# Rinoahu/SwiftOrtho

Hardware: AMD Instinct MI355X
Metric: M query-aa/s scanned all-vs-all (higher is better)
Workload: dtype u8/int16/int32 (5-bit packed residues, packed 16-bit score-only DP, int32 traced DP); 1 GPU; BASELINE config 3: 100000 synthetic proteins x 300 aa self-search, seed 11111011111, aa9, -M 120000000, -c 50000 (2 chunks), -e 1e-5, -v 500; query_aa=30007201, rows=1618760

## Files before the change

### swiftortho_amd/csrc/k_ungapq.hip

```cpp
#include "ungap1.h"

#define UQ_WAVES 16
#define UQ_RING 128
#define UQ_TBITS 12
#define UQ_QCAP 512
#define UQ_QSLOT (UQ_QCAP + 2 * U1_QPAD)
#define UQ_TILE 256
#define UQ_WAVE_BYTES (UQ_QSLOT + (1 << UQ_TBITS) / 4 + UQ_RING * 4 + UQ_RING * 4 + UQ_RING * 2 + UQ_TILE * 8)

__device__ __forceinline__ u32 bk_scan_max16(u32 x) {
    x = max(x, (u32)__builtin_amdgcn_update_dpp(0, (int)x, 0x111, 0xf, 0xf, true));
    x = max(x, (u32)__builtin_amdgcn_update_dpp(0, (int)x, 0x112, 0xf, 0xf, true));
    x = max(x, (u32)__builtin_amdgcn_update_dpp(0, (int)x, 0x114, 0xf, 0xf, true));
    x = max(x, (u32)__builtin_amdgcn_update_dpp(0, (int)x, 0x118, 0xf, 0xf, true));
    x = max(x, (u32)__builtin_amdgcn_update_dpp(0, (int)x, 0x142, 0xa, 0xf, false));
    x = max(x, (u32)__builtin_amdgcn_update_dpp(0, (int)x, 0x143, 0xc, 0xf, false));
    return x;
}

__device__ __forceinline__ u32 uq_slot(u32 g) { return (g * 2654435761u) >> (32 - UQ_TBITS); }

__global__ __launch_bounds__(256) void k_uq_first(const u32* __restrict__ qseg, u32 nqp, const u32* __restrict__ cs_hoff, u32 K, u32* __restrict__ qk) {
    const u32 q = blockIdx.x * 256u + threadIdx.x;
    if (q > nqp) return;
    const u32 x = qseg[q];
    u32 lo = 0, hi = K;
    while (lo < hi) {
        const u32 m = (lo + hi) >> 1;
        if (cs_hoff[m] < x) lo = m + 1;
        else hi = m;
    }
    qk[q] = lo;
}

template <bool BANDS, bool COUNT>
__global__ __launch_bounds__(64 * UQ_WAVES, 1) __attribute__((amdgpu_num_sgpr(96))) void k_ungapq(
    const u32* __restrict__ qseg , u32 nqp, u32 qa, const u32* __restrict__ qk, const u32* __restrict__ cs_hoff,
    const u32* __restrict__ cs_base, const u64* __restrict__ cs_kbase, const u32* __restrict__ dk32, int bp, int bd, int sh_q, int sh_qpos, int sh_diag, int diag_off, int rbs,
    int rsh_subj, int rsh_diag, int rdoff, const uint2* __restrict__ btab, u32 wait_n, const u8* __restrict__ q_scls, const u32* __restrict__ qoff,
    const u8* __restrict__ r_ug, const u32* __restrict__ roff, const signed char* __restrict__ b62g, u32* __restrict__ work_ctr, u32* __restrict__ shard_cnt,
    u64* __restrict__ p_qs, u64* __restrict__ p_sd, u64* __restrict__ p_ft, unsigned long long* __restrict__ group_count, u64* __restrict__ keys,
    u64* __restrict__ keys_sorted, u32* __restrict__ seg_end, unsigned long long* __restrict__ stat ) {
    constexpr int TSH = 3;
    constexpr u32 TBYTES = (u32)U1_ROWS << (8 + TSH);
    __shared__ __align__(16) unsigned char uq_smem[TBYTES + UQ_WAVES * UQ_WAVE_BYTES];
    const int lane = threadIdx.x & 63, w = threadIdx.x >> 6;
    for (u32 i = threadIdx.x; i < U1_ROWS * 32u * 32u; i += 64 * UQ_WAVES) {
        const u32 q = i >> 10, s = (i >> 5) & 31u, l = i & 31u;
        const int v = (q < SCLS_N && s < SCLS_N) ? (int)b62g[q * SCLS_N + s] : -100;
        *reinterpret_cast<short*>(uq_smem + ((q << 11) | (s << 6) | (l << 1))) = (short)v;
    }
    __syncthreads();
    unsigned char* wbase = uq_smem + TBYTES + (u32)w * UQ_WAVE_BYTES;
    u8* qslot = wbase;
    u32* tab = reinterpret_cast<u32*>(wbase + UQ_QSLOT);
    u32* ring_s = tab + (1 << UQ_TBITS) / 16;
    u32* ring_g = ring_s + UQ_RING;
    u16* ring_q = reinterpret_cast<u16*>(ring_g + UQ_RING);
    u32* mbase = reinterpret_cast<u32*>(ring_q + UQ_RING);
    u16* marks = reinterpret_cast<u16*>(mbase + UQ_TILE);
    u16* mqpos = marks + UQ_TILE;
    static_assert(UQ_TILE == 256, "tile_marks clears the marks with two words per lane");
    static_assert(U1_PCAP * 8 <= 7 * 64 && UQ_WAVES <= U1_ROWS, "pass buffer in a table row's tail");
    u64* s_pass = reinterpret_cast<u64*>(uq_smem + ((u32)w << 11) + 25 * 64);
    u16* s_passq = reinterpret_cast<u16*>(uq_smem + ((u32)w << 11) + 25 * 64 + U1_PCAP * 8);
    static_assert(U1_PCAP * 8 + U1_PCAP * 2 <= 7 * 64, "row tail");
    const unsigned long long lt = (1ull << lane) - 1ull;
    const u32 lanebase = (u32)(size_t)(__attribute__((address_space(3))) unsigned char*)uq_smem + ((u32)(lane & 31) << 1);
    const u32 pmask = (1u << bp) - 1u;
    const u32 dmask = (1u << bd) - 1u;
    u32 npb = 0, ngroups = 0;
    u32 ch_pos = 0, ch_end = 0;
    U1Track tr_unused;
    U1Count ct;
    ct.n = 0;
    ct.start();

    for (;;) {
        u32 qrel = 0;
        if (lane == 0) qrel = atomicAdd(work_ctr, 1u);
        qrel = (u32)__builtin_amdgcn_readfirstlane((int)qrel);
        if (qrel >= nqp) break;
        const u32 h0 = (u32)__builtin_amdgcn_readfirstlane((int)qseg[qrel]), h1 = (u32)__builtin_amdgcn_readfirstlane((int)qseg[qrel + 1]);
        if (h0 == h1) {
            if (lane == 0) seg_end[qrel] = h0;
            continue;
        }
        const u32 k0 = (u32)__builtin_amdgcn_readfirstlane((int)qk[qrel]), k1 = (u32)__builtin_amdgcn_readfirstlane((int)qk[qrel + 1]);
        const u32 gq = qa + qrel;
        const u32 qb0 = (u32)__builtin_amdgcn_readfirstlane((int)qoff[gq]);
        const int ql = (int)((u32)__builtin_amdgcn_readfirstlane((int)qoff[gq + 1]) - qb0);
        for (int i = lane * 16; i < UQ_QSLOT; i += 64 * 16) {
            const int p0 = i - U1_QPAD;
            uint4 v = make_uint4(0x18181818u, 0x18181818u, 0x18181818u, 0x18181818u);
            if (p0 >= 0 && p0 < ql) {
                v = u1_load16(q_scls + qb0 + (u32)p0);
                u32* d = reinterpret_cast<u32*>(&v);
#pragma unroll
                for (int k = 0; k < 4; ++k) {
                    const int nv = min(max(ql - p0 - 4 * k, 0), 4);
                    const u32 m = nv >= 4 ? 0xFFFFFFFFu : ((1u << (8 * nv)) - 1u);
                    d[k] = (d[k] & m) | (0x18181818u & ~m);
                }
                if (p0 == 0) d[0] = (d[0] & 0xFFFFFF00u) | 0x18u;
            }
            *reinterpret_cast<uint4*>(qslot + i) = v;
        }
        reinterpret_cast<uint4*>(tab)[lane] = make_uint4(0, 0, 0, 0);
        u1_wave_sync();
        const int qr_max = U1_QPAD + ql;
        const u64 kq = (u64)gq << sh_q;

        const u32 n = h1 - h0;
        u32 t_next = k0;
        u32 c_base = 0, c_qpos = 0;
        auto tile_marks = [&](u32 tb) {
            reinterpret_cast<u32*>(marks)[lane] = 0, reinterpret_cast<u32*>(marks)[64 + lane] = 0;
            u1_wave_sync();
            for (;;) {
                const u32 k = t_next + (u32)lane;
                u32 o = 0xFFFFFFFFu;
                if (k < k1) o = cs_hoff[k] - h0 - tb;
                const bool in = o < (u32)UQ_TILE;
                if (in) {
                    marks[o] = (u16)(o + 1u);
                    mbase[o] = cs_base[k] + h0;
                    mqpos[o] = (u16)((u32)(cs_kbase[k] >> sh_qpos) & pmask);
                }
                const u32 cnt = (u32)__popcll(__ballot(in));
                t_next += cnt;
                if (cnt < 64u) break;
            }
            u1_wave_sync();
        };
        auto gen_step = [&](u32 tb, u32 st, u32& c, u32& qpos, u32& o) -> bool {
            o = tb + 64u * st + (u32)lane;
            const u32 p1 = bk_scan_max16((u32)marks[64u * st + (u32)lane]);
            u32 base = c_base;
            qpos = c_qpos;
            if (p1) base = mbase[p1 - 1u], qpos = (u32)mqpos[p1 - 1u];
            c_base = (u32)__builtin_amdgcn_readlane((int)base, 63), c_qpos = (u32)__builtin_amdgcn_readlane((int)qpos, 63);
            c = 0xFFFFFFFFu;
            if (o >= n) return false;
            c = dk32[base + o];
            return (int)c >= 0;
        };
        for (u32 tb = 0; tb < n; tb += UQ_TILE) {
            tile_marks(tb);
            const u32 nst = (min(n - tb, (u32)UQ_TILE) + 63u) / 64u;
            for (u32 st = 0; st < nst; ++st) {
                u32 c, qpos, o;
                if (gen_step(tb, st, c, qpos, o)) {
                    const u32 t = uq_slot(c + qpos), sh = (t & 15u) * 2u;
                    const u32 old = atomicOr(&tab[t >> 4], 1u << sh);
                    if ((old >> sh) & 1u) atomicOr(&tab[t >> 4], 2u << sh);
                }
            }
        }
        u1_wave_sync();

        auto flush = [&]() {
            const u32 at = u1_reserve(npb, lane, ch_pos, ch_end, &shard_cnt[0], U1_CHUNK);
            if ((u32)lane < npb) {
                const u64 e = s_pass[lane];
                const u32 G = (u32)e, qp = (u32)s_passq[lane];
                u32 gsubj;
                int dlt;
                if (BANDS) {
                    const uint2 be = btab[G >> bd];
                    gsubj = be.x;
                    dlt = (int)(be.y - G);
                } else {
                    gsubj = G >> bd;
                    dlt = diag_off - (int)(G & dmask);
                }
                p_qs[at] = ((u64)gq << rbs) | gsubj;
                p_sd[at] = (e & 0xFFFFFFFF00000000ull) | (u64)(u32)dlt;
                p_ft[at] = ((u64)gsubj << rsh_subj) | ((u64)(u32)(rdoff - dlt) << rsh_diag) | ((u64)qp << sh_qpos);
            }
            npb = 0;
        };
        t_next = k0, c_base = 0, c_qpos = 0;
        u32 g_tb = 0, g_st = 0, g_nst = (min(n, (u32)UQ_TILE) + 63u) / 64u;
        tile_marks(0);
        bool more = true;
        u32 ns = 0;
        u32 rfront = 0, rback = 0;
        bool working = false;
        int qR = 0, qL = 0;
        i64 sR = 0, sL = 0;
        u32 hG = 0, hq = 0;
        pk16 S = {0, 0}, M = {0, 0};
        for (;;) {
            const unsigned long long idleb = __ballot(!working);
            if (idleb && ((u32)__popcll(idleb) >= wait_n || idleb == ~0ull)) {
                while (rback - rfront <= UQ_RING - 64u && more) {
                    u32 c, qpos, o;
                    const bool valid = gen_step(g_tb, g_st, c, qpos, o);
                    bool sing = false;
                    u32 G = 0;
                    if (valid) {
                        G = c + qpos;
                        const u32 t = uq_slot(G);
                        sing = ((tab[t >> 4] >> ((t & 15u) * 2u)) & 3u) == 1u;
                    }
                    const unsigned long long sb_ = __ballot(sing), kb_ = __ballot(valid && !sing);
                    if (valid && !sing) keys[h0 + ns + (u32)__popcll(kb_ & lt)] = kq + ((u64)qpos << sh_diag) + ((u64)qpos << sh_qpos) + ((u64)c << sh_diag);
                    ns += (u32)__popcll(kb_);
                    if (sing) {
                        u32 gsubj;
                        int dlt;
                        if (BANDS) {
                            const uint2 be = btab[G >> bd];
                            gsubj = be.x;
                            dlt = (int)(be.y - G);
                        } else {
                            gsubj = G >> bd;
                            dlt = diag_off - (int)(G & dmask);
                        }
                        const u32 slot = (rback + (u32)__popcll(sb_ & lt)) & (UQ_RING - 1);
                        ring_s[slot] = roff[gsubj] + (u32)((int)qpos + dlt);
                        ring_g[slot] = G;
                        ring_q[slot] = (u16)qpos;
                    }
                    rback += (u32)__popcll(sb_);
                    if (++g_st >= g_nst) {
                        g_st = 0, g_tb += UQ_TILE;
                        if (g_tb < n) {
                            g_nst = (min(n - g_tb, (u32)UQ_TILE) + 63u) / 64u;
                            tile_marks(g_tb);
                        } else {
                            more = false;
                        }
                    }
                }
                u1_wave_sync();
                const u32 avail = rback - rfront;
                if (!working) {
                    const u32 rk = (u32)__popcll(idleb & lt);
                    if (rk < avail) {
                        const u32 slot = (rfront + rk) & (UQ_RING - 1);
                        const u32 sa = ring_s[slot];
                        hG = ring_g[slot], hq = (u32)ring_q[slot];
                        qR = U1_QPAD + (int)hq, qL = qR - 16;
                        sR = (i64)sa, sL = (i64)sa - 16;
                        S = pk16{0, 0}, M = pk16{0, 0};
                        if (COUNT) ct.start();
                        working = true;
                    }
                }
                const u32 taken = min((u32)__popcll(idleb), avail);
                rfront += taken;
                ngroups += taken;
                u1_wave_sync();
            }
            if (!__ballot(working)) {
                if (!more && rback == rfront) break;
                continue;
            }
            bool fin = false;
            if (working) {
                const uint4 qr4 = u1_lds16(qslot, qR), ql4 = u1_lds16(qslot, qL);
                const uint4 sr4 = u1_load16(r_ug + sR), sl4 = u1_load16(r_ug + sL);
                const u32 msk = u1_step<TSH, false, COUNT>(qr4, ql4, sr4, sl4, lanebase, S, M, tr_unused, 0, ct);
                qR = min(qR + 16, qr_max), qL = max(qL - 16, 0);
                sR += 16, sL -= 16;
                fin = msk == 0xFFFFFFFFu;
            }
            {
                const int score = (int)M.x + (int)M.y;
                bool todo = fin && score >= MIN_UNGAP;
                for (;;) {
                    const unsigned long long pb = __ballot(todo);
                    if (!pb) break;
                    const u32 room = U1_PCAP - npb, rk = (u32)__popcll(pb & lt);
                    if (todo && rk < room) {
                        s_pass[npb + rk] = ((u64)(u32)score << 32) | hG;
                        s_passq[npb + rk] = (u16)hq;
                        todo = false;
                    }
                    npb += min((u32)__popcll(pb), room);
                    u1_wave_sync();
                    if (npb == U1_PCAP) {
                        flush();
                        u1_wave_sync();
                    }
                }
                if (fin) working = false;
            }
        }
        if (npb) {
            flush();
            u1_wave_sync();
        }
        if (lane == 0) seg_end[qrel] = h0 + ns;
        for (u32 i = h0 + ns + (u32)lane; i < h1; i += 64) keys_sorted[i] = ~0ull;
    }
    for (u32 i = ch_pos + (u32)lane; i < ch_end; i += 64) p_qs[i] = UG_REC_NONE, p_ft[i] = 0;
    if (lane == 0 && ngroups) atomicAdd(&group_count[0], (unsigned long long)ngroups);
    if (COUNT) {
        unsigned long long nst = ct.n;
#pragma unroll
        for (int o = 32; o > 0; o >>= 1) nst += __shfl_xor(nst, o);
        if (lane == 0) atomicAdd(&stat[0], nst), atomicAdd(&stat[1], (unsigned long long)ngroups);
    }
}

u32 ungapq_qcap() { return UQ_QCAP; }

void launch_ungapq(u32 ncu, const u32* qseg, u32 nqp, u32 qa, u32* qk, const u32* cs_hoff, const u32* cs_base, const u64* cs_kbase, u32 K, const u32* dk32,
                   const KeyLayout& kl, const KeyLayout& klr, const void* btab, const u8* q_scls, const u32* qoff, const u8* r_ug, const u32* roff, const signed char* b62g,
                   u32* work_ctr, u32* shard_cnt, u64* p_qs, u64* p_sd, u64* p_ft, unsigned long long* group_count, u64* keys, u64* keys_sorted, u32* seg_end,
                   unsigned long long* stat, hipStream_t st) {
    if (!nqp) return;
    hipLaunchKernelGGL(k_uq_first, dim3((nqp + 1 + 255) / 256), dim3(256), 0, st, qseg, nqp, cs_hoff, K, qk);
    static_assert(((size_t)U1_ROWS << 11) + (size_t)UQ_WAVES * UQ_WAVE_BYTES <= 160 * 1024, "LDS of a CU");
    const dim3 g(std::min<u32>(ncu, (nqp + UQ_WAVES - 1) / UQ_WAVES)), bl(64 * UQ_WAVES);
#define UQ_GO(B, CT)                                                                                                                                              \
    hipLaunchKernelGGL((k_ungapq<B, CT>), g, bl, 0, st, qseg, nqp, qa, qk, cs_hoff, cs_base, cs_kbase, dk32, kl.bp, kl.bd, kl.sh_q, kl.sh_qpos, kl.sh_diag, (int)kl.diag_off, klr.bs,  \
                       klr.sh_subj, klr.sh_diag, (int)klr.diag_off, (const uint2*)btab, U1_WAIT, q_scls, qoff, r_ug, roff, b62g, work_ctr, shard_cnt, p_qs, p_sd, p_ft,      \
                       group_count, keys, keys_sorted, seg_end, stat)
    if (stat) {
        if (btab) UQ_GO(true, true);
        else UQ_GO(false, true);
    } else if (btab) UQ_GO(true, false);
    else UQ_GO(false, false);
#undef UQ_GO
}
```

### swiftortho_amd/csrc/tune.h

```cpp
#pragma once
#include <cstdlib>

#define SOHIT_TUNE_TABLE(X)                                                                                                                                     \
                                                                                                                              \
    X(B, ug1, "SOHIT_UG1", 1, "bucketed passes: singleton groups to k_ungap1 (0: everything to k_ungap)")                                                     \
    X(B, ug1_chain, "SOHIT_UG1_CHAIN", 1, "... and the groups of two and more hits to k_ungap2 (0: to k_ungap, which then skips the singletons)")              \
    X(B, count_steps, "SOHIT_UG_COUNT", 0, "counting instances of the extension kernels: so_counters.ungap_steps, groups_single, groups_chain")                \
    X(B, ungapq, "SOHIT_UNGAPQ", 1, "sparse passes of queries up to 512 residues: hits alone on their diagonal by k_ungapq, a wave per query (0: every hit through the sorted keys)")     \
    X(B, ug_w32, "SOHIT_UG_W32", 1, "bucketed passes hand k_ungap the buckets' 32-bit words (0: 64-bit keys; no k_ungap1 then)")                               \
                                                                                                             \
    X(B, bucket, "SOHIT_BUCKET", 1, "bucketed diagonal binning (0: every pass on the sorted path)")                                                            \
    X(I, bucket_min, "SOHIT_BUCKET_MIN", 192, "hits per bucket below which a pass takes the sorted path (0: bucketed whenever possible)")                      \
    X(I, bucket_avg, "SOHIT_BUCKET_AVG", 2560, "average bucket size the band-range width is chosen for")                                                       \
    X(I, count_tab, "SOHIT_COUNT_TAB", 1, "bucketed passes: hits per (tile, range) from the range boundaries of the ordered index buckets when a batch brings a chunk two passes and more (0: always the counting pass over the entries; 2: always both, compared -- tests; 3: always)") \
    X(B, bucket_best, "SOHIT_BUCKET_BEST", 1, "best diagonal per subject by the per-bucket reduction (0: sort of the pass records)")                           \
    X(B, bands, "SOHIT_BANDS", 1, "diagonal bands follow the subjects' lengths (0: one band per subject)")                                                     \
    X(B, lk_wide, "SOHIT_LK_WIDE", 0, "8-byte index addends whatever the field widths")                                                                        \
    X(B, qclass, "SOHIT_QCLASS", 1, "queries of a batch in length-class order (0: file order)")                                                                \
    X(B, pass_merge, "SOHIT_PASS_MERGE", 1, "neighbouring length classes that take the sorted path anyway share one pass")                                     \
    X(B, ksc_lazy, "SOHIT_KSC_LAZY", 1, "k-mer orders computed for the queries that reach their frequency cap, when they do (a query below it keeps every window whatever the order; 0: for every query, with the batch)") \
    X(B, bounds_ahead, "SOHIT_BOUNDS_AHEAD", 1, "the next chunk's bucket bounds (k_bounds) on the side stream beside this chunk's seed stage (0: in front of its own)")     \
    X(I, segsort, "SOHIT_SEGSORT", 1, "sorted path: segmented sort of the keys inside each query (0: device-wide sort)")                                        \
    X(I, write_threads, "SOHIT_WRITE_THREADS", 48, "so_write_sc: formatter threads (at most the host's cores)")                                                                          \
                                                                                                                                 \
    X(I, cand_limit, "SOHIT_CAND_LIMIT", 0, "tests: candidate-store size at which a batch is split (0: 2^32 - 16)")                                            \
                                                                                                                                         \
    X(B, align_pk, "SOHIT_ALIGN_PK", 1, "packed 16-bit score-only aligner where the scores fit")                                                               \
    X(B, align_lane, "SOHIT_ALIGN_LANE", 1, "score-only rounds: one lane per alignment pair (k_align_lane) when no sequence reaches 4096 residues (0: k_align_pk)")            \
    X(I, align_lane_min, "SOHIT_ALIGN_LANE_MIN", 1 << 18, "... for rounds of at least this many packed tasks (below: k_align_pk; tests: 0)")                 \
    X(B, align_sort, "SOHIT_ALIGN_SORT", 1, "launch lists ordered by band rows")                                                                               \
    X(I, trace_wave_rows, "SOHIT_TRACE_WAVE_ROWS", 1024, "traceback: bands of this many rows and more are walked by a wave of their own (0: never)")         \
    X(I, trace_wave_max, "SOHIT_TRACE_WAVE_MAX", 32768, "... among the first this many positions of a launch list")                                            \
    X(I, spec, "SOHIT_SPEC", -1, "speculative traces in the first round: 0 off, 1 on, -1 from 2^21 tasks on")                                                  \
    X(D, spec_slack, "SOHIT_SPEC_SLACK", 1e6, "... the guess tests the ungapped score against expect x this (tests: 1e30 = every first-round task traced, 1e-30 = none)")          \
    X(I, spec_cap, "SOHIT_SPEC_CAP", -1, "tests: most speculative traces kept (-1: all)")                                                                      \
    X(I, trace_var_max, "SOHIT_TRACE_VAR_MAX", -1, "tests: trace words a launch list's own-size traces may take, and the fixed-stride slabs' budget (-1: 2^31 / 2^30)") \
    X(I, emit_parts, "SOHIT_EMIT_PARTS", 4, "... and otherwise")                                                                                               \
    X(I, emit_min_rows, "SOHIT_EMIT_MIN_ROWS", 1 << 18, "rows below which the emission is one part")                                                           \
    X(P, test_oom_phase2, "SOHIT_TEST_OOM_PHASE2", 0, "tests: phase 2 of the first batch fails once with an out-of-memory error")                              \
                                                                                                                                 \
    X(I, batch, "SOHIT_BATCH", 0, "queries per device batch (0: 131072, lowered when the candidate estimate asks)")                                            \
    X(I, max_hits, "SOHIT_MAX_HITS", 0, "seed hits per pass (0: 2^30)")                                                                                        \
    X(I, poison, "SOHIT_POISON", -1, "tests: byte every fresh device allocation is filled with (-1: none)")                                                    \
    X(B, hit_cache, "SOHIT_HIT_CACHE", 1, "one released result array is kept for the next search")                                                             \
    X(P, keep_cands, "SOHIT_KEEP_CANDS", 0, "tests: keep every query's candidate list (so_query_candidates)")                                                  \
    X(P, keep_masked, "SOHIT_KEEP_MASKED", 0, "tests: keep the masked queries (so_masked_query)")                                                              \
    X(I, mcl_scratch, "SOHIT_MCL_SCRATCH", -1, "tests: u32 words of expansion / convergence scratch per range of rows (-1: 2^28)")                             \
                                                                                      \
    X(T, orth_tier, "SOHIT_ORTH_TIER", 0, "tests: every run of query rows through one tier of k_orth_run wherever that tier can take it (0 = auto: by run length)") \
                                                                                                                                           \
    X(P, exact_threshold, "SOHIT_EXACT_THRESHOLD", 0, "threshold always by the sequential fp64 replay")                                                        \
    X(I, dir_max, "SOHIT_DIR_MAX", -1, "largest -M served by the bitmap + rank directory (-1: 2^31)")                                                          \
                                                                                                                                          \
    X(P, debug, "SOHIT_DEBUG", 0, "per-pass lines on stderr")                                                                                                  \
    X(P, debug_index, "SOHIT_DEBUG_INDEX", 0, "wall laps of the index build on stderr")

#define ORTH_WAVE_ROWS 64
#define ORTH_LDS_ROWS 1024
#define ORTH_LDS_TAXA 512
enum { ORTH_TIER_AUTO = 0, ORTH_TIER_WAVE = 1, ORTH_TIER_LDS = 2, ORTH_TIER_SCRATCH = 3 };
static inline int orth_tier_of(const char* v) {
    switch (v[0]) {
        case 'w': case '1': return ORTH_TIER_WAVE;
        case 'l': case '2': return ORTH_TIER_LDS;
        case 's': case '3': return ORTH_TIER_SCRATCH;
        default: return ORTH_TIER_AUTO;
    }
}

struct Tune {
#define X_B(f, d) bool f = (d) != 0;
#define X_I(f, d) long long f = (d);
#define X_D(f, d) double f = (d);
#define X_P(f, d) bool f = false;
#define X_T(f, d) int f = (d);
#define X(kind, field, env, dflt, text) X_##kind(field, dflt)
    SOHIT_TUNE_TABLE(X)
#undef X
#undef X_B
#undef X_I
#undef X_D
#undef X_P
#undef X_T
    void read() {
#define X_B(f, e) if (const char* v = getenv(e)) f = atoi(v) != 0;
#define X_I(f, e) if (const char* v = getenv(e)) f = strtoll(v, nullptr, 0);
#define X_D(f, e) if (const char* v = getenv(e)) f = atof(v);
#define X_P(f, e) f = getenv(e) != nullptr;
#define X_T(f, e) if (const char* v = getenv(e)) f = orth_tier_of(v);
#define X(kind, field, env, dflt, text) X_##kind(field, env)
        SOHIT_TUNE_TABLE(X)
#undef X
#undef X_B
#undef X_I
#undef X_D
#undef X_P
#undef X_T
    }
};

const Tune& tune();
void set_tune(const Tune* t);
```

Before: 671.2 M query-aa/s.

## Cache first-walk hit entries in registers and prefetch the second walk one step ahead

```diff
diff --git a/swiftortho_amd/csrc/k_ungapq.hip b/swiftortho_amd/csrc/k_ungapq.hip
--- a/swiftortho_amd/csrc/k_ungapq.hip
+++ b/swiftortho_amd/csrc/k_ungapq.hip
@@ -7,6 +7,9 @@
 #define UQ_QSLOT (UQ_QCAP + 2 * U1_QPAD)
 #define UQ_TILE 256
 #define UQ_WAVE_BYTES (UQ_QSLOT + (1 << UQ_TBITS) / 4 + UQ_RING * 4 + UQ_RING * 4 + UQ_RING * 2 + UQ_TILE * 8)
+#define UQ_CACHE 1024
+#define UQ_CSTEPS (UQ_CACHE / 64)
+static_assert(UQ_CACHE % UQ_TILE == 0 && UQ_CACHE > 0, "whole tiles");
 
 __device__ __forceinline__ u32 bk_scan_max16(u32 x) {
     x = max(x, (u32)__builtin_amdgcn_update_dpp(0, (int)x, 0x111, 0xf, 0xf, true));
@@ -17,6 +20,9 @@
     x = max(x, (u32)__builtin_amdgcn_update_dpp(0, (int)x, 0x143, 0xc, 0xf, false));
     return x;
 }
+
+typedef u32 uq_vc __attribute__((ext_vector_type(UQ_CSTEPS)));
+typedef u32 uq_vq __attribute__((ext_vector_type(UQ_CSTEPS / 2)));
 
 __device__ __forceinline__ u32 uq_slot(u32 g) { return (g * 2654435761u) >> (32 - UQ_TBITS); }
 
@@ -37,7 +43,7 @@
 __global__ __launch_bounds__(64 * UQ_WAVES, 1) __attribute__((amdgpu_num_sgpr(96))) void k_ungapq(
     const u32* __restrict__ qseg , u32 nqp, u32 qa, const u32* __restrict__ qk, const u32* __restrict__ cs_hoff,
     const u32* __restrict__ cs_base, const u64* __restrict__ cs_kbase, const u32* __restrict__ dk32, int bp, int bd, int sh_q, int sh_qpos, int sh_diag, int diag_off, int rbs,
-    int rsh_subj, int rsh_diag, int rdoff, const uint2* __restrict__ btab, u32 wait_n, const u8* __restrict__ q_scls, const u32* __restrict__ qoff,
+    int rsh_subj, int rsh_diag, int rdoff, const uint2* __restrict__ btab, u32 wait_n, u32 csteps , const u8* __restrict__ q_scls, const u32* __restrict__ qoff,
     const u8* __restrict__ r_ug, const u32* __restrict__ roff, const signed char* __restrict__ b62g, u32* __restrict__ work_ctr, u32* __restrict__ shard_cnt,
     u64* __restrict__ p_qs, u64* __restrict__ p_sd, u64* __restrict__ p_ft, unsigned long long* __restrict__ group_count, u64* __restrict__ keys,
     u64* __restrict__ keys_sorted, u32* __restrict__ seg_end, unsigned long long* __restrict__ stat ) {
@@ -133,25 +139,48 @@
             }
             u1_wave_sync();
         };
-        auto gen_step = [&](u32 tb, u32 st, u32& c, u32& qpos, u32& o) -> bool {
-            o = tb + 64u * st + (u32)lane;
+        auto owner = [&](u32 st, u32& base, u32& qpos) {
             const u32 p1 = bk_scan_max16((u32)marks[64u * st + (u32)lane]);
-            u32 base = c_base;
+            base = c_base;
             qpos = c_qpos;
             if (p1) base = mbase[p1 - 1u], qpos = (u32)mqpos[p1 - 1u];
             c_base = (u32)__builtin_amdgcn_readlane((int)base, 63), c_qpos = (u32)__builtin_amdgcn_readlane((int)qpos, 63);
+        };
+        auto gen_step = [&](u32 tb, u32 st, u32& c, u32& qpos) {
+            const u32 o = tb + 64u * st + (u32)lane;
+            u32 base;
+            owner(st, base, qpos);
             c = 0xFFFFFFFFu;
-            if (o >= n) return false;
-            c = dk32[base + o];
-            return (int)c >= 0;
-        };
+            if (o < n) c = dk32[base + o];
+        };
+        uq_vc cc = 0xFFFFFFFFu;
+        uq_vq cq = 0;
+        const u32 nsteps = (n + 63u) / 64u;
+        const u32 ncs = min(csteps, nsteps);
+        const u32 rg_tb = (csteps * 64u) & ~(u32)(UQ_TILE - 1);
+        u32 rg_tnext = k0, rg_base = 0, rg_qpos = 0;
         for (u32 tb = 0; tb < n; tb += UQ_TILE) {
+            if (tb == rg_tb) rg_tnext = t_next, rg_base = c_base, rg_qpos = c_qpos;
             tile_marks(tb);
             const u32 nst = (min(n - tb, (u32)UQ_TILE) + 63u) / 64u;
-            for (u32 st = 0; st < nst; ++st) {
-                u32 c, qpos, o;
-                if (gen_step(tb, st, c, qpos, o)) {
-                    const u32 t = uq_slot(c + qpos), sh = (t & 15u) * 2u;
+            u32 c4[4], q4[4];
+#pragma unroll
+            for (u32 st = 0; st < 4; ++st) {
+                c4[st] = 0xFFFFFFFFu, q4[st] = 0;
+                if (st < nst) gen_step(tb, st, c4[st], q4[st]);
+            }
+#pragma unroll
+            for (u32 t = 0; t < UQ_CSTEPS / 4; ++t) {
+                if (tb == t * UQ_TILE) {
+#pragma unroll
+                    for (u32 st = 0; st < 4; ++st) cc[4 * t + st] = c4[st];
+                    cq[2 * t] = q4[0] | (q4[1] << 16), cq[2 * t + 1] = q4[2] | (q4[3] << 16);
+                }
+            }
+#pragma unroll
+            for (u32 st = 0; st < 4; ++st) {
+                if ((int)c4[st] >= 0) {
+                    const u32 t = uq_slot(c4[st] + q4[st]), sh = (t & 15u) * 2u;
                     const u32 old = atomicOr(&tab[t >> 4], 1u << sh);
                     if ((old >> sh) & 1u) atomicOr(&tab[t >> 4], 2u << sh);
                 }
@@ -180,9 +209,49 @@
             }
             npb = 0;
         };
-        t_next = k0, c_base = 0, c_qpos = 0;
-        u32 g_tb = 0, g_st = 0, g_nst = (min(n, (u32)UQ_TILE) + 63u) / 64u;
-        tile_marks(0);
+        u32 p_c = 0xFFFFFFFFu, p_qpos = 0, p_ro = 0, p_ad = 0;
+        bool p_sing = false;
+        auto prepare = [&](u32 gs) {
+            u32 c, qpos;
+            if (gs < ncs) {
+                c = cc[gs];
+                const u32 w2 = cq[gs >> 1];
+                qpos = (gs & 1u) ? (w2 >> 16) : (w2 & 0xFFFFu);
+            } else {
+                const u32 st = gs & 3u, tb = (gs >> 2) * (u32)UQ_TILE;
+                if (st == 0 || gs == ncs) {
+                    if (gs == ncs) t_next = rg_tnext, c_base = rg_base, c_qpos = rg_qpos;
+                    tile_marks(tb);
+                    for (u32 s0 = 0; s0 < st; ++s0) {
+                        u32 b_, q_;
+                        owner(s0, b_, q_);
+                    }
+                }
+                gen_step(tb, st, c, qpos);
+            }
+            bool sing = false;
+            u32 ro = 0, ad = 0;
+            if ((int)c >= 0) {
+                const u32 G = c + qpos, t = uq_slot(G);
+                sing = ((tab[t >> 4] >> ((t & 15u) * 2u)) & 3u) == 1u;
+                if (sing) {
+                    u32 gsubj;
+                    int dlt;
+                    if (BANDS) {
+                        const uint2 be = btab[G >> bd];
+                        gsubj = be.x;
+                        dlt = (int)(be.y - G);
+                    } else {
+                        gsubj = G >> bd;
+                        dlt = diag_off - (int)(G & dmask);
+                    }
+                    ro = roff[gsubj], ad = (u32)((int)qpos + dlt);
+                }
+            }
+            p_c = c, p_qpos = qpos, p_ro = ro, p_ad = ad, p_sing = sing;
+        };
+        u32 g_s = 0;
+        prepare(0);
         bool more = true;
         u32 ns = 0;
         u32 rfront = 0, rback = 0;
@@ -195,44 +264,20 @@
             const unsigned long long idleb = __ballot(!working);
             if (idleb && ((u32)__popcll(idleb) >= wait_n || idleb == ~0ull)) {
                 while (rback - rfront <= UQ_RING - 64u && more) {
-                    u32 c, qpos, o;
-                    const bool valid = gen_step(g_tb, g_st, c, qpos, o);
-                    bool sing = false;
-                    u32 G = 0;
-                    if (valid) {
-                        G = c + qpos;
-                        const u32 t = uq_slot(G);
-                        sing = ((tab[t >> 4] >> ((t & 15u) * 2u)) & 3u) == 1u;
-                    }
+                    const u32 c = p_c, qpos = p_qpos, G = c + qpos;
+                    const bool valid = (int)c >= 0, sing = p_sing;
                     const unsigned long long sb_ = __ballot(sing), kb_ = __ballot(valid && !sing);
+                    if (sing) {
+                        const u32 slot = (rback + (u32)__popcll(sb_ & lt)) & (UQ_RING - 1);
+                        ring_s[slot] = p_ro + p_ad;
+                        ring_g[slot] = G;
+                        ring_q[slot] = (u16)qpos;
+                    }
+                    rback += (u32)__popcll(sb_);
+                    if (++g_s < nsteps) prepare(g_s);
+                    else more = false;
                     if (valid && !sing) keys[h0 + ns + (u32)__popcll(kb_ & lt)] = kq + ((u64)qpos << sh_diag) + ((u64)qpos << sh_qpos) + ((u64)c << sh_diag);
                     ns += (u32)__popcll(kb_);
-                    if (sing) {
-                        u32 gsubj;
-                        int dlt;
-                        if (BANDS) {
-                            const uint2 be = btab[G >> bd];
-                            gsubj = be.x;
-                            dlt = (int)(be.y - G);
-                        } else {
-                            gsubj = G >> bd;
-                            dlt = diag_off - (int)(G & dmask);
-                        }
-                        const u32 slot = (rback + (u32)__popcll(sb_ & lt)) & (UQ_RING - 1);
-                        ring_s[slot] = roff[gsubj] + (u32)((int)qpos + dlt);
-                        ring_g[slot] = G;
-                        ring_q[slot] = (u16)qpos;
-                    }
-                    rback += (u32)__popcll(sb_);
-                    if (++g_st >= g_nst) {
-                        g_st = 0, g_tb += UQ_TILE;
-                        if (g_tb < n) {
-                            g_nst = (min(n - g_tb, (u32)UQ_TILE) + 63u) / 64u;
-                            tile_marks(g_tb);
-                        } else {
-                            more = false;
-                        }
-                    }
                 }
                 u1_wave_sync();
                 const u32 avail = rback - rfront;
@@ -316,9 +361,11 @@
     hipLaunchKernelGGL(k_uq_first, dim3((nqp + 1 + 255) / 256), dim3(256), 0, st, qseg, nqp, cs_hoff, K, qk);
     static_assert(((size_t)U1_ROWS << 11) + (size_t)UQ_WAVES * UQ_WAVE_BYTES <= 160 * 1024, "LDS of a CU");
     const dim3 g(std::min<u32>(ncu, (nqp + UQ_WAVES - 1) / UQ_WAVES)), bl(64 * UQ_WAVES);
+    const long long uqc = tune().uq_cache;
+    const u32 csteps = uqc < 0 ? (u32)UQ_CSTEPS : (u32)std::min<long long>(uqc / 64, UQ_CSTEPS);
 #define UQ_GO(B, CT)                                                                                                                                              \
     hipLaunchKernelGGL((k_ungapq<B, CT>), g, bl, 0, st, qseg, nqp, qa, qk, cs_hoff, cs_base, cs_kbase, dk32, kl.bp, kl.bd, kl.sh_q, kl.sh_qpos, kl.sh_diag, (int)kl.diag_off, klr.bs,  \
-                       klr.sh_subj, klr.sh_diag, (int)klr.diag_off, (const uint2*)btab, U1_WAIT, q_scls, qoff, r_ug, roff, b62g, work_ctr, shard_cnt, p_qs, p_sd, p_ft,      \
+                       klr.sh_subj, klr.sh_diag, (int)klr.diag_off, (const uint2*)btab, U1_WAIT, csteps, q_scls, qoff, r_ug, roff, b62g, work_ctr, shard_cnt, p_qs, p_sd, p_ft,      \
                        group_count, keys, keys_sorted, seg_end, stat)
     if (stat) {
         if (btab) UQ_GO(true, true);
diff --git a/swiftortho_amd/csrc/tune.h b/swiftortho_amd/csrc/tune.h
--- a/swiftortho_amd/csrc/tune.h
+++ b/swiftortho_amd/csrc/tune.h
@@ -7,6 +7,7 @@
     X(B, ug1_chain, "SOHIT_UG1_CHAIN", 1, "... and the groups of two and more hits to k_ungap2 (0: to k_ungap, which then skips the singletons)")              \
     X(B, count_steps, "SOHIT_UG_COUNT", 0, "counting instances of the extension kernels: so_counters.ungap_steps, groups_single, groups_chain")                \
     X(B, ungapq, "SOHIT_UNGAPQ", 1, "sparse passes of queries up to 512 residues: hits alone on their diagonal by k_ungapq, a wave per query (0: every hit through the sorted keys)")     \
+    X(I, uq_cache, "SOHIT_UQ_CACHE", -1, "... its hit ordinals per query whose index entries stay in registers between the two walks, in steps of 64 (-1: the compiled 1024; 0: every entry read twice; tests move the boundary)") \
     X(B, ug_w32, "SOHIT_UG_W32", 1, "bucketed passes hand k_ungap the buckets' 32-bit words (0: 64-bit keys; no k_ungap1 then)")                               \
                                                                                                              \
     X(B, bucket, "SOHIT_BUCKET", 1, "bucketed diagonal binning (0: every pass on the sorted path)")                                                            \
```

Result: faster. 681.8 M query-aa/s, median of 6 (+1.6%).
